# mhnazeri/PMoE

Measured on AMD Instinct MI355X. Metric: samples/sec fwd+bwd, 256x256 RGB 4-expert PMoE, higher is better.
Workload: dtype bf16; 1 GPU; 4-expert MoE (PMoE experts), 256x256x3 x4 frames, batch 64/GPU, fwd+moe_loss+bwd, dropout 0.3; global_batch=64, parallelism=dp1

## Files before the change

### include/pmoe_hip.h

```cpp
#ifndef PMOE_HIP_H
#define PMOE_HIP_H
#include <stdint.h>
#ifdef __cplusplus
extern "C" {
#endif

#define PMOE_DT_BF16 0
#define PMOE_DT_F32 1

#define PMOE_ERR_ARG (-1)
#define PMOE_ERR_UNSUPPORTED (-2)

#define PMOE_ACT_NONE 0
#define PMOE_ACT_RELU 1
#define PMOE_ACT_ELU 2
#define PMOE_ACT_TANH 3
#define PMOE_ACT_SIGMOID 4

#define PMOE_RES_NONE 0
#define PMOE_RES_ADD 1
#define PMOE_RES_DRELU 2
#define PMOE_RES_DELU 3
#define PMOE_RES_DTANH 4
#define PMOE_RES_DSIGMOID 5
#define PMOE_RES_DBN 6
#define PMOE_RES_INBN 7

#define PMOE_ABI_VERSION 401
int pmoe_version(void);
const char* pmoe_error_string(int code);
int pmoe_abi_sizeof(int which);

typedef struct pmoe_conv_desc {
    const void* in;
    const void* w;
    void* out;
    const void* res;
    const float* bias;
    float* stats;
    int32_t n, h, w_, cin;
    int32_t ho, wo, cout, coutp;
    int32_t in_ld, in_coff, out_ld, out_coff, res_ld, res_coff;
    int32_t ipe;
    int32_t in_shared;
    int32_t ks, stride, pad, dilate;
    int32_t act, res_mode;
    float drop_p;
    uint64_t seed;
    int32_t dtype;
    int32_t w_fp8;
    float in_scale;
    const float* out_scale;
    int32_t in_fp8;
    const float* bn_coef;
    int32_t bn_ipe;
    int32_t shuffle_c;
} pmoe_conv_desc;

int pmoe_conv2d_igemm(const pmoe_conv_desc* d, void* stream);
// ... 282 lines not shown
```

### pmoe_amd/csrc/elementwise.hip

```cpp
#include "common.h"

template <typename T, int MODE>
__global__ void __launch_bounds__(256) colstats_kernel(const T* __restrict__ x, const T* __restrict__ dy,
                                                      const T* __restrict__ y, const float* __restrict__ mean,
                                                      const float* __restrict__ invstd, const float* __restrict__ scale,
                                                      const float* __restrict__ shift, long long rpe, int C, int ld,
                                                      int coff, int relu, float* __restrict__ part, int nparts,
                                                      float* __restrict__ shiftc, T* __restrict__ gmask) {
    constexpr int VE = 16 / (int)sizeof(T);
    const int CV = C / VE, RL = 256 / CV;
    const int tid = threadIdx.x, cv = tid % CV, rl = tid / CV;
    const int e = blockIdx.y, pi = blockIdx.x;
    const long long rpp = (rpe + nparts - 1) / nparts;
    long long r0 = (long long)pi * rpp, r1 = r0 + rpp;
    if (r1 > rpe) r1 = rpe;
    float s1[VE], s2[VE], mu[VE], is[VE], sc[VE], sh[VE];
    const bool remask = MODE && relu && !y;
#pragma unroll
    for (int i = 0; i < VE; ++i) {
        s1[i] = s2[i] = 0.f;
        mu[i] = MODE ? mean[e * C + cv * VE + i] : 0.f;
        is[i] = MODE ? invstd[e * C + cv * VE + i] : 0.f;
        sc[i] = remask ? scale[e * C + cv * VE + i] : 0.f;
        sh[i] = remask ? shift[e * C + cv * VE + i] : 0.f;
    }
    const size_t ebase = (size_t)e * rpe;
    float c0v[VE];
#pragma unroll
    for (int i = 0; i < VE; ++i) c0v[i] = 0.f;
    if (MODE == 0 && shiftc) {
        unpack16<T>(ldg16(x + ebase * ld + coff + cv * VE), c0v);
        if (pi == 0 && rl == 0) {
#pragma unroll
            for (int i = 0; i < VE; ++i) shiftc[e * C + cv * VE + i] = c0v[i];
        }
    }
    for (long long r = r0 + rl; r < r1; r += RL) {
        const size_t off = (ebase + r) * ld + coff + cv * VE;
        float xv[VE];
        unpack16<T>(ldg16(x + off), xv);
        if (MODE == 0) {
#pragma unroll
            for (int i = 0; i < VE; ++i) { const float d = xv[i] - c0v[i]; s1[i] += d; s2[i] += d * d; }
        } else {
            float gv[VE], yv[VE];
            unpack16<T>(ldg16(dy + off), gv);
            if (remask) {
#pragma unroll
                for (int i = 0; i < VE; ++i) gv[i] = ((xv[i] - mu[i]) * sc[i] + sh[i]) > 0.f ? gv[i] : 0.f;
            } else if (relu) {
                unpack16<T>(ldg16(y + off), yv);
#pragma unroll
                for (int i = 0; i < VE; ++i) gv[i] = yv[i] > 0.f ? gv[i] : 0.f;
            }
            if (gmask) stg16(gmask + off, pack16<T>(gv));
#pragma unroll
            for (int i = 0; i < VE; ++i) { s1[i] += gv[i]; s2[i] += gv[i] * (xv[i] - mu[i]) * is[i]; }
        }
    }
    __shared__ float red[2][256 * 8 / 1];
#pragma unroll
    for (int i = 0; i < VE; ++i) {
        red[0][rl * C + cv * VE + i] = s1[i];
        red[1][rl * C + cv * VE + i] = s2[i];
    }
    __syncthreads();
    for (int c = tid; c < 2 * C; c += 256) {
        const int which = c / C, cc = c % C;
        float s = 0.f;
        for (int k = 0; k < RL; ++k) s += red[which][k * C + cc];
        part[(((size_t)e * nparts + pi) * 2 + which) * C + cc] = s;
    }
}

template <typename T>
static int colstats_launch(const void* x, const void* dy, const void* y, const float* mean, const float* invstd,
                           const float* scale, const float* shift, long long rpe, int E, int C, int ld, int coff, int relu, float* part, int nparts, int mode,
                           float* shiftc, hipStream_t st, void* gmask = nullptr) {
    if (!one_vec_per_thread<T>(C) || nparts < 1 || rpe < 1 || E < 1) return PMOE_ERR_ARG;
    if (ld <= 0) { ld = C; coff = 0; }
    if (coff < 0 || !window_ok<T>(C, ld, coff)) return PMOE_ERR_ARG;
    dim3 grid(nparts, E), block(256);
    if (mode == 0)
        return launch<colstats_kernel<T, 0>, 0>(grid, block, 0, st, (const T*)x, nullptr, nullptr, nullptr, nullptr, nullptr,
                                                nullptr, rpe, C, ld, coff, 0, part, nparts, shiftc, nullptr);
    return launch<colstats_kernel<T, 1>, 0>(grid, block, 0, st, (const T*)x, (const T*)dy, (const T*)y, mean, invstd, scale,
                                            shift, rpe, C, ld, coff, relu, part, nparts, nullptr, (T*)gmask);
}

__global__ void __launch_bounds__(256) reduce_partials_kernel(const float* __restrict__ in, float* __restrict__ out,
// ... 99 lines not shown
                                                      unsigned char* __restrict__ y8, float in_scale) {
    constexpr int VE = 16 / (int)sizeof(T);
    const int CV = C / VE;
    const int e = blockIdx.y;
    const long long nvec = rpe * CV;
    const size_t ebase = (size_t)e * rpe * C;
    const long long i0 = (long long)blockIdx.x * 256 + threadIdx.x;
    const int cv = (int)(i0 % CV);
    float sc[VE], sh[VE], mu[VE];
#pragma unroll
    for (int k = 0; k < VE; ++k) {
        sc[k] = scale[e * C + cv * VE + k]; sh[k] = shift[e * C + cv * VE + k]; mu[k] = mean[e * C + cv * VE + k];
    }
    for (long long i = i0; i < nvec; i += (long long)gridDim.x * 256) {
        float xv[VE];
        const size_t off = ebase + (size_t)i * VE;
        unpack16<T>(ldg16(x + off), xv);
#pragma unroll
        for (int k = 0; k < VE; ++k) xv[k] = (xv[k] - mu[k]) * sc[k] + sh[k];
        if (res) {
            float rv[VE];
            unpack16<T>(ldg16(res + off), rv);
#pragma unroll
            for (int k = 0; k < VE; ++k) xv[k] += rv[k];
        }
        if (relu) {
#pragma unroll
            for (int k = 0; k < VE; ++k) xv[k] = fmaxf(xv[k], 0.f);
        }
        const size_t yoff = y_ld == C ? off : ((size_t)e * rpe + (size_t)(i >> log_cv)) * y_ld + y_coff + (size_t)cv * VE;
        const v4i pk = pack16<T>(xv);
        stg16(y + yoff, pk);
        if constexpr (sizeof(T) == 2) {
            if (y8) {
                float q[VE];
                unpack16<T>(pk, q);
                int w0 = 0, w1 = 0;
#pragma unroll
                for (int k = 0; k < VE; ++k) q[k] = fminf(fmaxf(q[k] * in_scale, -PMOE_FP8_MAX), PMOE_FP8_MAX);
                w0 = __builtin_amdgcn_cvt_pk_fp8_f32(q[0], q[1], w0, false);
                w0 = __builtin_amdgcn_cvt_pk_fp8_f32(q[2], q[3], w0, true);
                w1 = __builtin_amdgcn_cvt_pk_fp8_f32(q[4], q[5], w1, false);
                w1 = __builtin_amdgcn_cvt_pk_fp8_f32(q[6], q[7], w1, true);
                *reinterpret_cast<int2*>(y8 + ebase + (size_t)i * VE) = int2{w0, w1};
            }
        }
    }
}

template <typename T>
__global__ void __launch_bounds__(256) bn_bwd_apply_kernel(const T* __restrict__ dy, const T* __restrict__ y,
                                                          const T* __restrict__ x, const float* __restrict__ mean,
                                                          const float* __restrict__ invstd,
                                                          const float* __restrict__ scale, const float* __restrict__ shift,
                                                          const float* __restrict__ c1,
                                                          const float* __restrict__ c2, T* __restrict__ dx,
                                                          T* __restrict__ gm, long long rpe, int C, int relu) {
    constexpr int VE = 16 / (int)sizeof(T);
    const int CV = C / VE;
    const int e = blockIdx.y;
    const long long nvec = rpe * CV;
    const size_t ebase = (size_t)e * rpe * C;
    const long long i0 = (long long)blockIdx.x * 256 + threadIdx.x;
    const int cv = (int)(threadIdx.x & (CV - 1));
    float A[VE], Bx[VE], K[VE], sc[VE], sh[VE], mu[VE];
#pragma unroll
    for (int k = 0; k < VE; ++k) {
        const int c = e * C + cv * VE + k;
        sc[k] = scale[c];
        sh[k] = shift ? shift[c] : 0.f;
        mu[k] = mean[c];
        A[k] = sc[k];
        Bx[k] = -sc[k] * invstd[c] * c2[c];
        K[k] = -sc[k] * c1[c];
    }
    const bool remask = relu && !y;
    for (long long i = i0; i < nvec; i += (long long)gridDim.x * 256) {
        const size_t off = ebase + (size_t)i * VE;
        float gv[VE], xv[VE], o[VE];
        unpack16<T>(ldg16(dy + off), gv);
        unpack16<T>(ldg16(x + off), xv);
        if (remask) {
#pragma unroll
            for (int k = 0; k < VE; ++k) gv[k] = ((xv[k] - mu[k]) * sc[k] + sh[k]) > 0.f ? gv[k] : 0.f;
        } else if (relu) {
            float yv[VE];
            unpack16<T>(ldg16(y + off), yv);
#pragma unroll
            for (int k = 0; k < VE; ++k) gv[k] = yv[k] > 0.f ? gv[k] : 0.f;
        }
#pragma unroll
        for (int k = 0; k < VE; ++k) o[k] = gv[k] * A[k] + ((xv[k] - mu[k]) * Bx[k] + K[k]);
        stg16(dx + off, pack16<T>(o));
        if (gm) stg16(gm + off, pack16<T>(gv));
    }
}

template <typename T>
__global__ void __launch_bounds__(256) bn_apply_pool2_kernel(const T* __restrict__ x, T* __restrict__ y, T* __restrict__ pooled,
                                                            const float* __restrict__ scale, const float* __restrict__ shift,
                                                            const float* __restrict__ mean, int ipe, int H, int W, int C, int relu,
                                                            int y_ld, int y_coff) {
    constexpr int VE = 16 / (int)sizeof(T);
    const int CV = C / VE;
    const int e = blockIdx.y, Ho = H / 2, Wo = W / 2;
    const long long nq = (long long)ipe * Ho * Wo * CV;
    const long long i0 = (long long)blockIdx.x * 256 + threadIdx.x;
    const int cv = (int)(i0 % CV);
    float sc[VE], sh[VE], mu[VE];
#pragma unroll
    for (int k = 0; k < VE; ++k) {
        sc[k] = scale[e * C + cv * VE + k]; sh[k] = shift[e * C + cv * VE + k]; mu[k] = mean[e * C + cv * VE + k];
    }
    const size_t rpe = (size_t)ipe * H * W;
    for (long long i = i0; i < nq; i += (long long)gridDim.x * 256) {
        long long t = i / CV;
        const int ox = (int)(t % Wo); t /= Wo;
// ... 389 lines not shown

template <typename T>
__global__ void __launch_bounds__(256) act_bwd_kernel(const T* __restrict__ dy, const T* __restrict__ y, T* __restrict__ dx,
                                                     long long nvec, int act, float drop_p) {
    constexpr int VE = 16 / (int)sizeof(T);
    const float keep_scale = drop_p > 0.f ? 1.f / (1.f - drop_p) : 1.f;
    const int mode = act == PMOE_ACT_ELU ? PMOE_RES_DELU : act == PMOE_ACT_TANH ? PMOE_RES_DTANH : PMOE_RES_DSIGMOID;
    for (long long i = (long long)blockIdx.x * 256 + threadIdx.x; i < nvec; i += (long long)gridDim.x * 256) {
        float g[VE], yv[VE];
        unpack16<T>(ldg16(dy + i * VE), g);
        unpack16<T>(ldg16(y + i * VE), yv);
#pragma unroll
        for (int k = 0; k < VE; ++k) {
            if (act == PMOE_ACT_NONE) g[k] = (drop_p > 0.f && yv[k] == 0.f) ? 0.f : g[k] * keep_scale;
            else if (act == PMOE_ACT_RELU) g[k] = yv[k] > 0.f ? g[k] * keep_scale : 0.f;
            else g[k] = (drop_p > 0.f && yv[k] == 0.f) ? 0.f : g[k] * act_deriv_from_output(mode, yv[k] * (1.f / keep_scale)) * keep_scale;
        }
        stg16(dx + i * VE, pack16<T>(g));
    }
}

extern "C" {

int pmoe_colstats(const void* x, int64_t rows_per_expert, int32_t E, int32_t C, int32_t ld, int32_t coff, float* part,
                  int32_t nparts, float* shiftc, int32_t dtype, void* stream) {
    DISPATCH_DT(dtype, return colstats_launch<T>(x, nullptr, nullptr, nullptr, nullptr, nullptr, nullptr, rows_per_expert, E, C, ld, coff,
                                                 0, part, nparts, 0, shiftc, (hipStream_t)stream));
}

int pmoe_bn_bwd_reduce(const void* dy, const void* y, const void* x, const float* mean, const float* invstd,
                       const float* scale, const float* shift, int64_t rows_per_expert, int32_t E, int32_t C, int32_t relu, float* part, int32_t nparts,
                       void* gmask_out, int32_t dtype, void* stream) {
    if (relu && !y && (!scale || !shift)) return PMOE_ERR_ARG;
    DISPATCH_DT(dtype, return colstats_launch<T>(x, dy, y, mean, invstd, scale, shift, rows_per_expert, E, C, C, 0, relu, part,
                                                 nparts, 1, nullptr, (hipStream_t)stream, gmask_out));
}

int pmoe_reduce_partials(const float* part_in, float* part_out, int32_t E, int32_t nin, int32_t nout, int32_t width,
                         void* stream) {
    if (nin < 1 || nout < 1 || width < 1) return PMOE_ERR_ARG;
    return launch<reduce_partials_kernel, 0>(dim3(nout, E), dim3(256), 0, (hipStream_t)stream, part_in, part_out, nin, nout, width);
}

int pmoe_bn_finalize(const float* part, int32_t nparts, int64_t count, const void* const* gamma_ptrs,
                     const void* const* beta_ptrs, void* const* rmean_ptrs, void* const* rvar_ptrs, float momentum,
                     float eps, int32_t training, float* scale, float* shift, float* mean, float* invstd, int32_t E,
                     int32_t C, const float* shiftc, void* stream) {
    if (!training && (!rmean_ptrs || !rvar_ptrs)) return PMOE_ERR_ARG;
    return launch<bn_finalize_kernel, 0>(dim3((C + FIN_CH - 1) / FIN_CH, E), dim3(FIN_CH * FIN_LANES), 0, (hipStream_t)stream,
                                         part, nparts, (long long)count, (const float* const*)gamma_ptrs,
                                         (const float* const*)beta_ptrs, (float* const*)rmean_ptrs, (float* const*)rvar_ptrs,
                                         momentum, eps, training, scale, shift, mean, invstd, C, shiftc);
}

int pmoe_bn_bwd_finalize(const float* part, int32_t nparts, int64_t count, float* dgamma, float* dbeta, float* c1,
                         float* c2, int32_t E, int32_t C, void* stream) {
    return launch<bn_bwd_finalize_kernel, 0>(dim3((C + FIN_CH - 1) / FIN_CH, E), dim3(FIN_CH * FIN_LANES), 0, (hipStream_t)stream,
                                             part, nparts, (long long)count, dgamma, dbeta, c1, c2, C);
}

int pmoe_bn_apply(const void* x, const void* res, void* y, const float* scale, const float* shift, const float* mean,
                  int64_t rows_per_expert, int32_t E, int32_t C, int32_t relu, int32_t y_ld, int32_t y_coff, int32_t dtype,
                  void* y_fp8, float in_scale, void* stream) {
    DISPATCH_DT(dtype, {
        if (!one_vec_per_thread<T>(C)) return PMOE_ERR_ARG;
        if (y_ld <= 0) { y_ld = C; y_coff = 0; }
        if (y_fp8 && (dtype != PMOE_DT_BF16 || y_ld != C)) return PMOE_ERR_ARG;
        if (!window_ok<T>(C, y_ld, y_coff)) return PMOE_ERR_ARG;
        const int CV = C / VecOf<T>::N;
        return launch<bn_apply_kernel<T>, 0>(dim3(grid_for(rows_per_expert * CV, 2048), E), dim3(256), 0, (hipStream_t)stream,
                                             (const T*)x, (const T*)res, (T*)y, scale, shift, mean, (long long)rows_per_expert, C,
                                             relu, y_ld, y_coff, ilog2_exact(CV), (unsigned char*)y_fp8, in_scale);
    });
}

int pmoe_bn_apply_pool2(const void* x, void* y, void* pooled, const float* scale, const float* shift, const float* mean,
                        int32_t ipe, int32_t H, int32_t W, int32_t E, int32_t C, int32_t relu, int32_t y_ld, int32_t y_coff,
                        int32_t dtype, void* stream) {
    if (!x || !y || !pooled || ipe < 1 || E < 1 || H < 2 || W < 2 || (H & 1) || (W & 1)) return PMOE_ERR_ARG;
    DISPATCH_DT(dtype, {
        if (!one_vec_per_thread<T>(C)) return PMOE_ERR_ARG;
        if (y_ld <= 0) { y_ld = C; y_coff = 0; }
        if (!window_ok<T>(C, y_ld, y_coff)) return PMOE_ERR_ARG;
        const long long nq = (long long)ipe * (H / 2) * (W / 2) * (C / VecOf<T>::N);
        return launch<bn_apply_pool2_kernel<T>, 0>(dim3(grid_for(nq, 2048), E), dim3(256), 0, (hipStream_t)stream, (const T*)x,
                                                   (T*)y, (T*)pooled, scale, shift, mean, ipe, H, W, C, relu, y_ld, y_coff);
    });
}

int pmoe_bn_bwd_apply(const void* dy, const void* y, const void* x, const float* mean, const float* invstd,
                      const float* scale, const float* shift, const float* c1, const float* c2, void* dx, void* gmask_out,
                      int64_t rows_per_expert, int32_t E, int32_t C, int32_t relu, int32_t dtype, void* stream) {
    DISPATCH_DT(dtype, {
        if (!one_vec_per_thread<T>(C)) return PMOE_ERR_ARG;
        const long long nvec = rows_per_expert * (C / VecOf<T>::N);
        int cap = 1024 / (E > 0 ? E : 1);
        cap = cap < 64 ? 64 : cap;
        return launch<bn_bwd_apply_kernel<T>, 0>(dim3(grid_for(nvec, cap), E), dim3(256), 0, (hipStream_t)stream, (const T*)dy,
                                                 (const T*)y, (const T*)x, mean, invstd, scale, shift, c1, c2, (T*)dx,
                                                 (T*)gmask_out, (long long)rows_per_expert, C, relu);
    });
}

int pmoe_act_fwd(const void* x, void* y, int64_t n, int32_t act, float drop_p, uint64_t seed, int32_t dtype, void* stream) {
    if (!x || !y || n <= 0 || act < PMOE_ACT_NONE || act > PMOE_ACT_SIGMOID || drop_p < 0.f || drop_p >= 1.f) return PMOE_ERR_ARG;
    DISPATCH_DT(dtype, {
        constexpr int VE = VecOf<T>::N;
        if (n % VE) return PMOE_ERR_ARG;
        return launch<act_fwd_kernel<T>, 0>(dim3(grid_for(n / VE, 4096)), dim3(256), 0, (hipStream_t)stream, (const T*)x, (T*)y,
                                            (long long)(n / VE), act, drop_p, (unsigned long long)seed);
    });
}

int pmoe_act_bwd(const void* dy, const void* y, void* dx, int64_t n, int32_t act, float drop_p, int32_t dtype, void* stream) {
    if (!dy || !y || !dx || n <= 0 || act < PMOE_ACT_NONE || act > PMOE_ACT_SIGMOID || drop_p < 0.f || drop_p >= 1.f) return PMOE_ERR_ARG;
    DISPATCH_DT(dtype, {
        constexpr int VE = VecOf<T>::N;
        if (n % VE) return PMOE_ERR_ARG;
        return launch<act_bwd_kernel<T>, 0>(dim3(grid_for(n / VE, 4096)), dim3(256), 0, (hipStream_t)stream, (const T*)dy,
                                            (const T*)y, (T*)dx, (long long)(n / VE), act, drop_p);
    });
}

int pmoe_maxpool3s2_fwd(const void* x, void* y, uint8_t* argmax, int32_t N, int32_t H, int32_t W, int32_t C,
                        int32_t dtype, void* stream) {
// ... 118 lines not shown
```

### pmoe_amd/engine.py

```python
import collections
import itertools
import os

import torch
import torch.distributed as dist

from . import hip, ops
from .model import blocks as B
from .parallel import BucketedAllReduce

F32 = torch.float32


def r16(c):
    return (c + 15) // 16 * 16


def r64(c):
    return (c + 63) // 64 * 64


class Var:
    __slots__ = ("t", "coff", "c", "g", "needs_grad", "act", "drop_p", "base", "gap_part", "bn_src", "bn_part", "f8", "bn_defer",
                 "bn_fused", "pending_bn")

    def __init__(self, t, c=None, coff=0, needs_grad=False, base=None):
        self.t, self.coff, self.c = t, coff, (c if c is not None else t.shape[-1])
        self.g, self.needs_grad, self.act, self.drop_p, self.base = None, needs_grad, hip.ACT_NONE, 0.0, base
        self.gap_part = None
        self.bn_src = None
        self.bn_part = None
        self.f8 = None
        self.bn_defer = False
        self.bn_fused = None
        self.pending_bn = None

    @property
    def grad(self):
        return self.base.g if self.base is not None else self.g

    def set_grad(self, g):
        if (self.base if self.base is not None else self).bn_part is not None:
            raise RuntimeError("relu(BatchNorm(z)) whose backward reductions came out of its consumer's data gradient "
                               "(PMOE_RES_DBN) takes exactly one consumer; a second gradient contribution arrived")
        if self.base is not None:
            self.base.g = g
        else:
            self.g = g

    def window(self, coff, c):
        v = Var(self.t, c, coff, self.needs_grad, base=self if self.base is None else self.base)
        return v


PackSinks = collections.namedtuple("PackSinks", "gen by_param")


class GroupedConv:
    scatter_grads = None
    route_bias = True

    def __init__(self, eng, name, weights, biases, cin, cout, ks, stride, pad):
        self.eng, self.name = eng, name
        self.weights, self.biases = weights, biases
        self.cin, self.cout, self.ks, self.stride, self.pad = cin, cout, ks, stride, pad
        self.cinp, self.coutp, self.cout_st = r16(cin), r64(cout), r16(cout)
        self.dg_rows, self.dg_red = r64(cin), r16(cout)
        self.taps = ks * ks
# ... 508 lines not shown
    def _bn_coeffs(self, layer, rpe, part=None, nparts=0, z=None, shiftc=None):
        E, C_ = self.E, layer.C
        coef = self._last_coef = torch.empty(4, E, C_, dtype=F32, device=self.dev)
        mean, invstd, scale, shift = coef[0], coef[1], coef[2], coef[3]
        if self.training:
            if part is None:
                nparts = self._nparts(rpe)
                part = torch.empty(E, nparts, 2, C_, dtype=F32, device=self.dev)
                shiftc = torch.empty(E, C_, dtype=F32, device=self.dev)
                ops.colstats(rpe, z.t, E, C_, part, nparts, shiftc=shiftc)
            part, nparts = self._fold_parts(part, nparts, 2 * C_, cap=2048)
            ops.bn_finalize(part, nparts, rpe, self._tab("gamma", layer), self._tab("beta", layer),
                            self._tab("rm", layer), self._tab("rv", layer), layer.momentum, layer.eps, True, scale,
                            shift, mean, invstd, E, C_, shiftc)
            self._bn_touched.append(layer)
        else:
            ops.bn_finalize(scale, 0, rpe, self._tab("gamma", layer), self._tab("beta", layer), self._tab("rm", layer),
                            self._tab("rv", layer), layer.momentum, layer.eps, False, scale, shift, mean, invstd, E, C_)
        return scale, shift, mean, invstd

    def _bn(self, z, layer, relu, res=None, stats=None, out=None, out_coff=0, want_gap=False, want_f8=False, pool_to=None):
        E, C_ = self.E, layer.C
        n, h, w, _ = z.t.shape
        rpe = self.B * h * w
        if stats is not None and stats.shape[2] != C_:
            raise RuntimeError("fused stats width mismatch")
        scale, shift, mean, invstd = self._bn_coeffs(layer, rpe, stats, stats.shape[0] // E if stats is not None else 0, z)
        if out is None:
            y = Var(torch.empty_like(z.t))
        elif self.taping:
            y = Var(out.t, C_, out_coff)
        else:
            y = out.window(out_coff, C_)
        ops.set_meta(name=layer.name, bytes=z.t.numel() * z.t.element_size() * (3 if res is not None else 2))
        if want_gap and res is None and out is None:
            nparts = self._gap_parts(h * w)
            part = torch.empty(n, nparts, C_, dtype=F32, device=self.dev)
            ops.bn_apply_gap(z.t, y.t, scale, shift, mean, part, nparts, self.B, relu)
            y.gap_part = (part, nparts)
        elif pool_to is not None and res is None:
            ops.bn_apply_pool2(z.t, y.t, pool_to, scale, shift, mean, self.B, E, C_, relu, y_coff=y.coff)
        else:
            if want_f8 and out is None and self.dtype == torch.bfloat16:
                y.f8 = torch.empty(y.t.shape, dtype=torch.uint8, device=self.dev)
            ops.bn_apply(z.t, res.t if res is not None else None, y.t, scale, shift, mean, rpe, E, C_, relu, y_coff=y.coff,
                         y_fp8=y.f8, in_scale=self.fp8_in_scale)
        if self.debug_acts is not None and relu:
            self.debug_acts[layer.name] = (y.t, y.coff, C_)
        if relu and res is None and out is None and self.taping and self.training and self.dtype == torch.bfloat16 and z.needs_grad:
            y.bn_src = (z, layer, self._last_coef, rpe)
        y.needs_grad = z.needs_grad or layer.trainable or (res is not None and res.needs_grad)
        if out is not None and y.needs_grad:
            out.needs_grad = True
        if self.taping and y.needs_grad:
            train = self.training
            self.tape.append(lambda: self._bn_bwd(z, layer, y, res, relu, scale, shift, mean, invstd, rpe, train))
        return y

    def _bn_bwd(self, z, layer, y, res, relu, scale, shift, mean, invstd, rpe, train):
        dy = y.grad
        if self.debug_grads is not None and dy is not None:
            self.debug_grads[layer.name] = dy.detach().clone()
        ysrc = y.t if (res is not None or not relu) else None
        if dy is None:
            return
        E, C_ = self.E, layer.C
        nb = z.t.numel() * z.t.element_size()
        if y.bn_part is not None:
            part, nparts = y.bn_part
            if part.shape[2] != C_:
                raise RuntimeError("BatchNorm reductions from the data-gradient epilogue: channel count mismatch")
            part, nparts = self._fold_parts(part.view(E, nparts, 2 * C_), nparts, 2 * C_, cap=2048)
            c1, c2 = self._bn_bwd_finalize(layer, part, nparts, rpe, train)
            if z.needs_grad:
                if z.grad is not None:
                    raise RuntimeError("BN input consumed twice")
                if z.bn_defer:
                    z.bn_fused = (dy, y.bn_src[2], c1, c2)
                    z.set_grad(dy)
                    return
                dz = torch.empty_like(z.t)
                ops.set_meta(name=layer.name, bytes=nb * 3)
                ops.bn_bwd_apply(dy, None, z.t, mean, invstd, scale, shift, c1, c2, dz, None, rpe, E, C_, False)
                z.set_grad(dz)
            return
        nparts = self._nparts(rpe)
        part = torch.empty(E, nparts, 2, C_, dtype=F32, device=self.dev)
        want_res = res is not None and res.needs_grad
        gm = torch.empty_like(z.t) if (want_res and relu and ysrc is not None) else None
        ops.set_meta(name=layer.name, bytes=nb * ((3 if ysrc is not None else 2) + (gm is not None)))
        ops.bn_bwd_reduce(dy, ysrc, z.t, mean, invstd, scale, shift, rpe, E, C_, relu, part, nparts, gmask=gm)
        part, nparts = self._fold_parts(part, nparts, 2 * C_, cap=2048)
        c1, c2 = self._bn_bwd_finalize(layer, part, nparts, rpe, train)
        dz = torch.empty_like(z.t) if z.needs_grad else None
        if gm is not None:
            if dz is not None:
                ops.set_meta(name=layer.name, bytes=nb * 3)
                ops.bn_bwd_apply(gm, None, z.t, mean, invstd, scale, shift, c1, c2, dz, None, rpe, E, C_, False)
        else:
            gm = torch.empty_like(z.t) if want_res else None
            if dz is None and gm is None:
                return
            if dz is None:
                dz = torch.empty_like(z.t)
            ops.set_meta(name=layer.name, bytes=nb * (2 + (ysrc is not None) + 1 + (gm is not None)))
            ops.bn_bwd_apply(dy, ysrc, z.t, mean, invstd, scale, shift, c1, c2, dz, gm, rpe, E, C_, relu)
        if self.debug_grads is not None:
            self.debug_grads[layer.name + ":dz"] = dz.detach().clone()
            self.debug_grads[layer.name + ":stats"] = (mean.clone(), invstd.clone(), c1.clone(), c2.clone())
        if z.needs_grad:
            if z.grad is not None:
                raise RuntimeError("BN input consumed twice")
            z.set_grad(dz)
        if want_res:
            if res.grad is not None:
                raise RuntimeError("residual gradient slot already filled")
            res.set_grad(gm)

    def _bn_bwd_finalize(self, layer, part, nparts, rpe, train, out=None):
        E, C_ = self.E, layer.C
        c1, c2 = out or (torch.empty(E, C_, dtype=F32, device=self.dev) for _ in range(2))
        dgamma, dbeta, store = self._bn_grad_views(layer)
        ops.bn_bwd_finalize(part, nparts, rpe, dgamma, dbeta, c1, c2, E, C_)
        if store is not None:
            store()
        if not train:
            c1.zero_()
            c2.zero_()
        return c1, c2

    def _bn_grad_views(self, layer):
        return (self._grad_slot("gamma", layer).view(self.E, layer.C), self._grad_slot("beta", layer).view(self.E, layer.C),
                None)

    def _stem_tail(self, z2, stats):
        E, C_ = self.E, self.bn_c2.C
        n, h, w, _ = z2.t.shape
        rpe = self.B * h * w
        sc2, sh2, mu2, is2 = self._bn_coeffs(self.bn_c2, rpe, stats, stats.shape[0] // E if stats is not None else 0, z2)
# ... 537 lines not shown
```

### pmoe_amd/hip.py

```python
import ctypes as C
import os
from pathlib import Path

import torch

_LIB_PATH = Path(os.environ.get("PMOE_HIP_LIB") or Path(__file__).resolve().parent / "libpmoe_hip.so")
_lib = None

ABI_VERSION = 401
DT_BF16, DT_F32 = 0, 1
ACT_NONE, ACT_RELU, ACT_ELU, ACT_TANH, ACT_SIGMOID = 0, 1, 2, 3, 4
RES_NONE, RES_ADD, RES_DRELU, RES_DELU, RES_DTANH, RES_DSIGMOID, RES_DBN, RES_INBN = 0, 1, 2, 3, 4, 5, 6, 7
ERR_ARG, ERR_UNSUPPORTED = -1, -2
RES_OF_ACT = {ACT_RELU: RES_DRELU, ACT_ELU: RES_DELU, ACT_TANH: RES_DTANH, ACT_SIGMOID: RES_DSIGMOID}
ACT_BY_NAME = {"relu": ACT_RELU, "elu": ACT_ELU, "tanh": ACT_TANH, "sigmoid": ACT_SIGMOID}

_TORCH_DT = {torch.bfloat16: DT_BF16, torch.float32: DT_F32}


class HipUnavailable(RuntimeError):
    pass


class ConvDesc(C.Structure):
    _fields_ = [
        ("in_", C.c_void_p), ("w", C.c_void_p), ("out", C.c_void_p), ("res", C.c_void_p),
        ("bias", C.c_void_p), ("stats", C.c_void_p),
        ("n", C.c_int32), ("h", C.c_int32), ("w_", C.c_int32), ("cin", C.c_int32),
        ("ho", C.c_int32), ("wo", C.c_int32), ("cout", C.c_int32), ("coutp", C.c_int32),
        ("in_ld", C.c_int32), ("in_coff", C.c_int32), ("out_ld", C.c_int32), ("out_coff", C.c_int32),
        ("res_ld", C.c_int32), ("res_coff", C.c_int32),
        ("ipe", C.c_int32), ("in_shared", C.c_int32),
        ("ks", C.c_int32), ("stride", C.c_int32), ("pad", C.c_int32), ("dilate", C.c_int32),
        ("act", C.c_int32), ("res_mode", C.c_int32),
        ("drop_p", C.c_float), ("seed", C.c_uint64), ("dtype", C.c_int32),
        ("w_fp8", C.c_int32), ("in_scale", C.c_float), ("out_scale", C.c_void_p),
        ("in_fp8", C.c_int32), ("bn_coef", C.c_void_p), ("bn_ipe", C.c_int32), ("shuffle_c", C.c_int32),
    ]


class WgradDesc(C.Structure):
    _fields_ = [
        ("x", C.c_void_p), ("dy", C.c_void_p), ("dw_ws", C.c_void_p),
        ("n", C.c_int32), ("h", C.c_int32), ("w_", C.c_int32), ("cin", C.c_int32), ("cinp", C.c_int32),
        ("ho", C.c_int32), ("wo", C.c_int32), ("cout", C.c_int32), ("coutp", C.c_int32),
        ("x_ld", C.c_int32), ("x_coff", C.c_int32), ("dy_ld", C.c_int32), ("dy_coff", C.c_int32),
# ... 210 lines not shown
```

### pmoe_amd/ops.py

```python
import ctypes as C

import torch

from . import hip
from .hip import ConvDesc, WgradDesc, check, dt, load, ptr, stream_ptr


def _round_up(v, m):
    return (v + m - 1) // m * m


def conv_out_size(h, ks, stride, pad):
    return (h + 2 * pad - ks) // stride + 1


def _nhwc(t, name):
    if t.dim() != 4:
        raise ValueError(f"{name}: expected NHWC [N,H,W,C], got shape {tuple(t.shape)}")
    return t.shape


def _conv_desc(n, h, w_, ho, wo, cin, cout, coutp, ipe, ks, stride, pad, dtype, *, dilate=False, in_shared=False, in_ld=0,
               in_coff=0, out_ld=0, out_coff=0, res_mode=hip.RES_NONE, res_ld=0, res_coff=0, act=hip.ACT_NONE, drop_p=0.0, seed=0,
               w_fp8=False, in_fp8=False, in_scale=1.0, bn_ipe=0, shuffle2_c=0):
# ... 271 lines not shown
                                stream_ptr()), "pmoe_pack_bias")


def act_fwd(x, y, act, drop_p=0.0, seed=0):
    check(load().pmoe_act_fwd(ptr(x, "x"), ptr(y, "y", x.dtype), x.numel(), act, float(drop_p), int(seed), dt(x), stream_ptr()),
          "pmoe_act_fwd")


def act_bwd(dy, y, dx, act, drop_p=0.0):
    check(load().pmoe_act_bwd(ptr(dy, "dy"), ptr(y, "y", dy.dtype), ptr(dx, "dx", dy.dtype), dy.numel(), act, float(drop_p),
                              dt(dy), stream_ptr()), "pmoe_act_bwd")


def colstats(x2d_rows_per_expert, x, E, C_, part, nparts, ld=None, coff=0, shiftc=None):
    check(load().pmoe_colstats(ptr(x, "x"), x2d_rows_per_expert, E, C_, ld if ld is not None else x.shape[-1], coff,
                               ptr(part, "part", torch.float32), nparts, ptr(shiftc, "shiftc", torch.float32), dt(x),
                               stream_ptr()), "pmoe_colstats")


def reduce_partials(part_in, part_out, E, nin, nout, width):
    check(load().pmoe_reduce_partials(ptr(part_in, "part_in", torch.float32), ptr(part_out, "part_out", torch.float32),
                                      E, nin, nout, width, stream_ptr()), "pmoe_reduce_partials")


def bn_finalize(part, nparts, count, gamma_tab, beta_tab, rmean_tab, rvar_tab, momentum, eps, training, scale, shift,
                mean, invstd, E, C_, shiftc=None):
    f32 = torch.float32
    check(load().pmoe_bn_finalize(ptr(part, "part", f32), nparts, count, ptr(gamma_tab), ptr(beta_tab), ptr(rmean_tab),
                                  ptr(rvar_tab), momentum, eps, int(training), ptr(scale, "scale", f32),
                                  ptr(shift, "shift", f32), ptr(mean, "mean", f32), ptr(invstd, "invstd", f32), E, C_,
                                  ptr(shiftc, "shiftc", f32), stream_ptr()), "pmoe_bn_finalize")


def bn_apply(x, res, y, scale, shift, mean, rpe, E, C_, relu, y_coff=0, y_fp8=None, in_scale=1.0):
    if y_fp8 is not None and (y_fp8.dtype != torch.uint8 or y_fp8.shape != y.shape):
        raise ValueError("bn_apply: y_fp8 must be a uint8 tensor of y's shape")
    check(load().pmoe_bn_apply(ptr(x, "x"), ptr(res, "res", x.dtype), ptr(y, "y", x.dtype), ptr(scale), ptr(shift),
                               ptr(mean, "mean", torch.float32), rpe,
                               E, C_, int(relu), y.shape[-1], y_coff, dt(x), ptr(y_fp8, "y_fp8", torch.uint8),
                               float(in_scale), stream_ptr()), "pmoe_bn_apply")


def bn_apply_pool2(x, y, pooled, scale, shift, mean, ipe, E, C_, relu, y_coff=0):
    n, h, w_, c = _nhwc(x, "x")
    if c != C_ or tuple(pooled.shape) != (n, h // 2, w_ // 2, C_) or tuple(y.shape[:3]) != (n, h, w_) or n != E * ipe:
        raise ValueError("bn_apply_pool2: x [E*ipe,H,W,C], y [E*ipe,H,W,ld], pooled [E*ipe,H/2,W/2,C]")
    check(load().pmoe_bn_apply_pool2(ptr(x, "x"), ptr(y, "y", x.dtype), ptr(pooled, "pooled", x.dtype), ptr(scale), ptr(shift),
                                     ptr(mean, "mean", torch.float32), ipe, h, w_, E, C_, int(relu), y.shape[-1], y_coff, dt(x),
                                     stream_ptr()), "pmoe_bn_apply_pool2")


def bn_bwd_reduce(dy, y, x, mean, invstd, scale, shift, rpe, E, C_, relu, part, nparts, gmask=None):
    check(load().pmoe_bn_bwd_reduce(ptr(dy, "dy"), ptr(y, "y", dy.dtype), ptr(x, "x", dy.dtype), ptr(mean), ptr(invstd),
                                    ptr(scale), ptr(shift), rpe, E, C_, int(relu), ptr(part, "part", torch.float32), nparts,
                                    ptr(gmask, "gmask", dy.dtype), dt(dy), stream_ptr()), "pmoe_bn_bwd_reduce")


def bn_bwd_finalize(part, nparts, count, dgamma, dbeta, c1, c2, E, C_):
    check(load().pmoe_bn_bwd_finalize(ptr(part), nparts, count, ptr(dgamma), ptr(dbeta), ptr(c1), ptr(c2), E, C_,
                                      stream_ptr()), "pmoe_bn_bwd_finalize")


def bn_bwd_apply(dy, y, x, mean, invstd, scale, shift, c1, c2, dx, gmask, rpe, E, C_, relu):
    check(load().pmoe_bn_bwd_apply(ptr(dy, "dy"), ptr(y, "y", dy.dtype), ptr(x, "x", dy.dtype), ptr(mean), ptr(invstd),
                                   ptr(scale), ptr(shift), ptr(c1), ptr(c2), ptr(dx, "dx", dy.dtype), ptr(gmask, "gmask", dy.dtype),
                                   rpe, E, C_, int(relu), dt(dy), stream_ptr()), "pmoe_bn_bwd_apply")


def stem_tail_stats(z2, sc2, sh2, mu2, part, nparts, E, ipe, shiftc=None, part_x=None):
    n, h, w_, c = _nhwc(z2, "z2")
    check(load().pmoe_stem_tail_stats(ptr(z2, "z2"), ptr(sc2), ptr(sh2), ptr(mu2), ptr(part, "part", torch.float32), nparts,
                                      ptr(shiftc, "shiftc", torch.float32), ptr(part_x, "part_x", torch.float32), E, ipe,
                                      h, w_, c, dt(z2), stream_ptr()), "pmoe_stem_tail_stats")


def _consts12(consts):
    return (C.c_void_p * 12)(*[t.data_ptr() if t is not None else None for t in consts])


def stem_tail_pooled(y, dpool, argmax, consts, part4, nparts, E):
    n, ho, wo, c = _nhwc(y, "y")
    check(load().pmoe_stem_tail_pooled(ptr(y, "y"), ptr(dpool, "dpool", y.dtype), ptr(argmax, "argmax", torch.uint8),
                                       _consts12(consts), ptr(part4, "part4", torch.float32), nparts, E,
                                       (n // E) * ho * wo, c, dt(y), stream_ptr()), "pmoe_stem_tail_pooled")


def stem_tail_combine(part4, np4, part_x, npx, consts, count, out1, out2, E, c):
    f32 = torch.float32
    check(load().pmoe_stem_tail_combine(ptr(part4, "part4", f32), np4, ptr(part_x, "part_x", f32), npx, _consts12(consts),
                                        count, ptr(out1, "out1", f32), ptr(out2, "out2", f32), E, c, stream_ptr()),
          "pmoe_stem_tail_combine")


def stem_tail_pool(z2, y, argmax, sc2, sh2, sc1, sh1, mu2, mu1, ipe):
    n, h, w_, c = _nhwc(z2, "z2")
    check(load().pmoe_stem_tail_pool(ptr(z2, "z2"), ptr(y, "y", z2.dtype), ptr(argmax, "argmax", torch.uint8), ptr(sc2),
                                     ptr(sh2), ptr(sc1), ptr(sh1), ptr(mu2), ptr(mu1), n, ipe, h, w_, c, dt(z2), stream_ptr()),
          "pmoe_stem_tail_pool")

# ... 397 lines not shown
```

Baseline: 1911 samples/s.

## Store ReLU masks as packed bits for residual BN backward

For residual BN+ReLU layers in bf16 training, the forward apply kernel now writes a 1-bit-per-channel ReLU mask, and the backward reduce and apply kernels read that mask instead of reloading the full bf16 output. This cuts backward memory traffic for the y tensor to one sixteenth, at the cost of an extra small write in forward. The colstats backward loop is also unrolled over four rows to batch loads and hide latency.

```diff
diff --git a/include/pmoe_hip.h b/include/pmoe_hip.h
--- a/include/pmoe_hip.h
+++ b/include/pmoe_hip.h
@@ -25,6 +25,8 @@
 #define PMOE_RES_DSIGMOID 5
 #define PMOE_RES_DBN 6
 #define PMOE_RES_INBN 7
+
+#define PMOE_RELU_BITS 2
 
 #define PMOE_ABI_VERSION 401
 int pmoe_version(void);
diff --git a/pmoe_amd/csrc/elementwise.hip b/pmoe_amd/csrc/elementwise.hip
--- a/pmoe_amd/csrc/elementwise.hip
+++ b/pmoe_amd/csrc/elementwise.hip
@@ -1,4 +1,6 @@
 #include "common.h"
+
+constexpr int COLSTATS_ROWS = 4;
 
 template <typename T, int MODE>
 __global__ void __launch_bounds__(256) colstats_kernel(const T* __restrict__ x, const T* __restrict__ dy,
@@ -35,27 +37,55 @@
             for (int i = 0; i < VE; ++i) shiftc[e * C + cv * VE + i] = c0v[i];
         }
     }
-    for (long long r = r0 + rl; r < r1; r += RL) {
-        const size_t off = (ebase + r) * ld + coff + cv * VE;
-        float xv[VE];
-        unpack16<T>(ldg16(x + off), xv);
-        if (MODE == 0) {
+    if constexpr (MODE == 0) {
+        for (long long r = r0 + rl; r < r1; r += RL) {
+            float xv[VE];
+            unpack16<T>(ldg16(x + (ebase + r) * ld + coff + cv * VE), xv);
 #pragma unroll
             for (int i = 0; i < VE; ++i) { const float d = xv[i] - c0v[i]; s1[i] += d; s2[i] += d * d; }
-        } else {
-            float gv[VE], yv[VE];
-            unpack16<T>(ldg16(dy + off), gv);
+        }
+    } else {
+        const bool bits = relu == PMOE_RELU_BITS, from_y = relu && !remask && !bits;
+        const unsigned char* __restrict__ yb = reinterpret_cast<const unsigned char*>(y);
+        auto add_row = [&](const v4i& xr, const v4i& gr, const v4i& yr, unsigned mb, size_t off) {
+            float xv[VE], gv[VE];
+            unpack16<T>(xr, xv);
+            unpack16<T>(gr, gv);
             if (remask) {
 #pragma unroll
                 for (int i = 0; i < VE; ++i) gv[i] = ((xv[i] - mu[i]) * sc[i] + sh[i]) > 0.f ? gv[i] : 0.f;
+            } else if (bits) {
+#pragma unroll
+                for (int i = 0; i < VE; ++i) gv[i] = ((mb >> i) & 1u) ? gv[i] : 0.f;
             } else if (relu) {
-                unpack16<T>(ldg16(y + off), yv);
+                float yv[VE];
+                unpack16<T>(yr, yv);
 #pragma unroll
                 for (int i = 0; i < VE; ++i) gv[i] = yv[i] > 0.f ? gv[i] : 0.f;
             }
             if (gmask) stg16(gmask + off, pack16<T>(gv));
 #pragma unroll
             for (int i = 0; i < VE; ++i) { s1[i] += gv[i]; s2[i] += gv[i] * (xv[i] - mu[i]) * is[i]; }
+        };
+        long long r = r0 + rl;
+        for (; r + (long long)(COLSTATS_ROWS - 1) * RL < r1; r += (long long)COLSTATS_ROWS * RL) {
+            v4i xr[COLSTATS_ROWS], gr[COLSTATS_ROWS], yr[COLSTATS_ROWS];
+            unsigned mb[COLSTATS_ROWS];
+#pragma unroll
+            for (int u = 0; u < COLSTATS_ROWS; ++u) {
+                const size_t row = ebase + r + (long long)u * RL, off = row * ld + coff + cv * VE;
+                xr[u] = ldg16(x + off);
+                gr[u] = ldg16(dy + off);
+                yr[u] = from_y ? ldg16(y + off) : v4i{0, 0, 0, 0};
+                mb[u] = bits ? yb[row * CV + cv] : 0u;
+            }
+#pragma unroll
+            for (int u = 0; u < COLSTATS_ROWS; ++u)
+                add_row(xr[u], gr[u], yr[u], mb[u], (ebase + r + (long long)u * RL) * ld + coff + cv * VE);
+        }
+        for (; r < r1; r += RL) {
+            const size_t row = ebase + r, off = row * ld + coff + cv * VE;
+            add_row(ldg16(x + off), ldg16(dy + off), from_y ? ldg16(y + off) : v4i{0, 0, 0, 0}, bits ? yb[row * CV + cv] : 0u, off);
         }
     }
     __shared__ float red[2][256 * 8 / 1];
@@ -221,7 +251,14 @@
         const v4i pk = pack16<T>(xv);
         stg16(y + yoff, pk);
         if constexpr (sizeof(T) == 2) {
-            if (y8) {
+            if (y8 && relu == PMOE_RELU_BITS) {
+                float q[VE];
+                unpack16<T>(pk, q);
+                unsigned m = 0;
+#pragma unroll
+                for (int k = 0; k < VE; ++k) m |= (q[k] > 0.f ? 1u : 0u) << k;
+                y8[(size_t)e * nvec + (size_t)i] = (unsigned char)m;
+            } else if (y8) {
                 float q[VE];
                 unpack16<T>(pk, q);
                 int w0 = 0, w1 = 0;
@@ -263,7 +300,8 @@
         Bx[k] = -sc[k] * invstd[c] * c2[c];
         K[k] = -sc[k] * c1[c];
     }
-    const bool remask = relu && !y;
+    const bool remask = relu && !y, bits = relu == PMOE_RELU_BITS;
+    const unsigned char* __restrict__ yb = reinterpret_cast<const unsigned char*>(y);
     for (long long i = i0; i < nvec; i += (long long)gridDim.x * 256) {
         const size_t off = ebase + (size_t)i * VE;
         float gv[VE], xv[VE], o[VE];
@@ -272,6 +310,10 @@
         if (remask) {
 #pragma unroll
             for (int k = 0; k < VE; ++k) gv[k] = ((xv[k] - mu[k]) * sc[k] + sh[k]) > 0.f ? gv[k] : 0.f;
+        } else if (bits) {
+            const unsigned m = yb[(size_t)e * nvec + (size_t)i];
+#pragma unroll
+            for (int k = 0; k < VE; ++k) gv[k] = ((m >> k) & 1u) ? gv[k] : 0.f;
         } else if (relu) {
             float yv[VE];
             unpack16<T>(ldg16(y + off), yv);
@@ -727,6 +769,7 @@
                        const float* scale, const float* shift, int64_t rows_per_expert, int32_t E, int32_t C, int32_t relu, float* part, int32_t nparts,
                        void* gmask_out, int32_t dtype, void* stream) {
     if (relu && !y && (!scale || !shift)) return PMOE_ERR_ARG;
+    if (relu == PMOE_RELU_BITS && (!y || dtype != PMOE_DT_BF16)) return PMOE_ERR_ARG;
     DISPATCH_DT(dtype, return colstats_launch<T>(x, dy, y, mean, invstd, scale, shift, rows_per_expert, E, C, C, 0, relu, part,
                                                  nparts, 1, nullptr, (hipStream_t)stream, gmask_out));
 }
@@ -761,6 +804,7 @@
         if (!one_vec_per_thread<T>(C)) return PMOE_ERR_ARG;
         if (y_ld <= 0) { y_ld = C; y_coff = 0; }
         if (y_fp8 && (dtype != PMOE_DT_BF16 || y_ld != C)) return PMOE_ERR_ARG;
+        if (relu == PMOE_RELU_BITS && !y_fp8) return PMOE_ERR_ARG;
         if (!window_ok<T>(C, y_ld, y_coff)) return PMOE_ERR_ARG;
         const int CV = C / VecOf<T>::N;
         return launch<bn_apply_kernel<T>, 0>(dim3(grid_for(rows_per_expert * CV, 2048), E), dim3(256), 0, (hipStream_t)stream,
@@ -786,6 +830,7 @@
 int pmoe_bn_bwd_apply(const void* dy, const void* y, const void* x, const float* mean, const float* invstd,
                       const float* scale, const float* shift, const float* c1, const float* c2, void* dx, void* gmask_out,
                       int64_t rows_per_expert, int32_t E, int32_t C, int32_t relu, int32_t dtype, void* stream) {
+    if (relu == PMOE_RELU_BITS && (!y || dtype != PMOE_DT_BF16)) return PMOE_ERR_ARG;
     DISPATCH_DT(dtype, {
         if (!one_vec_per_thread<T>(C)) return PMOE_ERR_ARG;
         const long long nvec = rows_per_expert * (C / VecOf<T>::N);
diff --git a/pmoe_amd/engine.py b/pmoe_amd/engine.py
--- a/pmoe_amd/engine.py
+++ b/pmoe_amd/engine.py
@@ -22,7 +22,7 @@
 
 class Var:
     __slots__ = ("t", "coff", "c", "g", "needs_grad", "act", "drop_p", "base", "gap_part", "bn_src", "bn_part", "f8", "bn_defer",
-                 "bn_fused", "pending_bn")
+                 "bn_fused", "pending_bn", "relu_bits")
 
     def __init__(self, t, c=None, coff=0, needs_grad=False, base=None):
         self.t, self.coff, self.c = t, coff, (c if c is not None else t.shape[-1])
@@ -34,6 +34,7 @@
         self.bn_defer = False
         self.bn_fused = None
         self.pending_bn = None
+        self.relu_bits = None
 
     @property
     def grad(self):
@@ -608,6 +609,7 @@
             y = Var(out.t, C_, out_coff)
         else:
             y = out.window(out_coff, C_)
+        needs_grad = z.needs_grad or layer.trainable or (res is not None and res.needs_grad)
         ops.set_meta(name=layer.name, bytes=z.t.numel() * z.t.element_size() * (3 if res is not None else 2))
         if want_gap and res is None and out is None:
             nparts = self._gap_parts(h * w)
@@ -619,13 +621,16 @@
         else:
             if want_f8 and out is None and self.dtype == torch.bfloat16:
                 y.f8 = torch.empty(y.t.shape, dtype=torch.uint8, device=self.dev)
+            if (res is not None and relu and self.taping and self.training and self.dtype == torch.bfloat16 and out is None
+                    and y.f8 is None and needs_grad):
+                y.relu_bits = torch.empty(y.t.shape[:-1] + (C_ // 8,), dtype=torch.uint8, device=self.dev)
             ops.bn_apply(z.t, res.t if res is not None else None, y.t, scale, shift, mean, rpe, E, C_, relu, y_coff=y.coff,
-                         y_fp8=y.f8, in_scale=self.fp8_in_scale)
+                         y_fp8=y.f8, in_scale=self.fp8_in_scale, relu_bits=y.relu_bits)
         if self.debug_acts is not None and relu:
             self.debug_acts[layer.name] = (y.t, y.coff, C_)
         if relu and res is None and out is None and self.taping and self.training and self.dtype == torch.bfloat16 and z.needs_grad:
             y.bn_src = (z, layer, self._last_coef, rpe)
-        y.needs_grad = z.needs_grad or layer.trainable or (res is not None and res.needs_grad)
+        y.needs_grad = needs_grad
         if out is not None and y.needs_grad:
             out.needs_grad = True
         if self.taping and y.needs_grad:
@@ -638,6 +643,8 @@
         if self.debug_grads is not None and dy is not None:
             self.debug_grads[layer.name] = dy.detach().clone()
         ysrc = y.t if (res is not None or not relu) else None
+        ybits = y.relu_bits if (ysrc is not None and relu) else None
+        yarg = ysrc if ybits is None else None
         if dy is None:
             return
         E, C_ = self.E, layer.C
@@ -664,8 +671,9 @@
         part = torch.empty(E, nparts, 2, C_, dtype=F32, device=self.dev)
         want_res = res is not None and res.needs_grad
         gm = torch.empty_like(z.t) if (want_res and relu and ysrc is not None) else None
-        ops.set_meta(name=layer.name, bytes=nb * ((3 if ysrc is not None else 2) + (gm is not None)))
-        ops.bn_bwd_reduce(dy, ysrc, z.t, mean, invstd, scale, shift, rpe, E, C_, relu, part, nparts, gmask=gm)
+        ybytes = 0 if ysrc is None else nb if ybits is None else ybits.numel()
+        ops.set_meta(name=layer.name, bytes=nb * (2 + (gm is not None)) + ybytes)
+        ops.bn_bwd_reduce(dy, yarg, z.t, mean, invstd, scale, shift, rpe, E, C_, relu, part, nparts, gmask=gm, y_bits=ybits)
         part, nparts = self._fold_parts(part, nparts, 2 * C_, cap=2048)
         c1, c2 = self._bn_bwd_finalize(layer, part, nparts, rpe, train)
         dz = torch.empty_like(z.t) if z.needs_grad else None
@@ -679,8 +687,8 @@
                 return
             if dz is None:
                 dz = torch.empty_like(z.t)
-            ops.set_meta(name=layer.name, bytes=nb * (2 + (ysrc is not None) + 1 + (gm is not None)))
-            ops.bn_bwd_apply(dy, ysrc, z.t, mean, invstd, scale, shift, c1, c2, dz, gm, rpe, E, C_, relu)
+            ops.set_meta(name=layer.name, bytes=nb * (3 + (gm is not None)) + ybytes)
+            ops.bn_bwd_apply(dy, yarg, z.t, mean, invstd, scale, shift, c1, c2, dz, gm, rpe, E, C_, relu, y_bits=ybits)
         if self.debug_grads is not None:
             self.debug_grads[layer.name + ":dz"] = dz.detach().clone()
             self.debug_grads[layer.name + ":stats"] = (mean.clone(), invstd.clone(), c1.clone(), c2.clone())
diff --git a/pmoe_amd/hip.py b/pmoe_amd/hip.py
--- a/pmoe_amd/hip.py
+++ b/pmoe_amd/hip.py
@@ -12,6 +12,7 @@
 ACT_NONE, ACT_RELU, ACT_ELU, ACT_TANH, ACT_SIGMOID = 0, 1, 2, 3, 4
 RES_NONE, RES_ADD, RES_DRELU, RES_DELU, RES_DTANH, RES_DSIGMOID, RES_DBN, RES_INBN = 0, 1, 2, 3, 4, 5, 6, 7
 ERR_ARG, ERR_UNSUPPORTED = -1, -2
+RELU_BITS = 2
 RES_OF_ACT = {ACT_RELU: RES_DRELU, ACT_ELU: RES_DELU, ACT_TANH: RES_DTANH, ACT_SIGMOID: RES_DSIGMOID}
 ACT_BY_NAME = {"relu": ACT_RELU, "elu": ACT_ELU, "tanh": ACT_TANH, "sigmoid": ACT_SIGMOID}
 
diff --git a/pmoe_amd/ops.py b/pmoe_amd/ops.py
--- a/pmoe_amd/ops.py
+++ b/pmoe_amd/ops.py
@@ -327,12 +327,27 @@
                                   ptr(shiftc, "shiftc", f32), stream_ptr()), "pmoe_bn_finalize")
 
 
-def bn_apply(x, res, y, scale, shift, mean, rpe, E, C_, relu, y_coff=0, y_fp8=None, in_scale=1.0):
+def _relu_arg(relu, bits, other, what):
+    if bits is None:
+        return int(relu)
+    if other is not None or not relu:
+        raise ValueError(f"{what}: the ReLU bits go with relu=True and take the place of the other tensor of their slot")
+    if bits.dtype != torch.uint8:
+        raise ValueError(f"{what}: the ReLU bits are a uint8 tensor")
+    return hip.RELU_BITS
+
+
+def bn_apply(x, res, y, scale, shift, mean, rpe, E, C_, relu, y_coff=0, y_fp8=None, in_scale=1.0, relu_bits=None):
     if y_fp8 is not None and (y_fp8.dtype != torch.uint8 or y_fp8.shape != y.shape):
         raise ValueError("bn_apply: y_fp8 must be a uint8 tensor of y's shape")
+    relu_arg = _relu_arg(relu, relu_bits, y_fp8, "bn_apply")
+    if relu_bits is not None:
+        if x.dtype != torch.bfloat16 or tuple(relu_bits.shape) != tuple(y.shape[:-1]) + (C_ // 8,):
+            raise ValueError("bn_apply: relu_bits needs bfloat16 data and a uint8 tensor of shape y.shape[:-1] + (C // 8,)")
+        y_fp8 = relu_bits
     check(load().pmoe_bn_apply(ptr(x, "x"), ptr(res, "res", x.dtype), ptr(y, "y", x.dtype), ptr(scale), ptr(shift),
                                ptr(mean, "mean", torch.float32), rpe,
-                               E, C_, int(relu), y.shape[-1], y_coff, dt(x), ptr(y_fp8, "y_fp8", torch.uint8),
+                               E, C_, relu_arg, y.shape[-1], y_coff, dt(x), ptr(y_fp8, "y_fp8", torch.uint8),
                                float(in_scale), stream_ptr()), "pmoe_bn_apply")
 
 
@@ -345,9 +360,19 @@
                                      stream_ptr()), "pmoe_bn_apply_pool2")
 
 
-def bn_bwd_reduce(dy, y, x, mean, invstd, scale, shift, rpe, E, C_, relu, part, nparts, gmask=None):
-    check(load().pmoe_bn_bwd_reduce(ptr(dy, "dy"), ptr(y, "y", dy.dtype), ptr(x, "x", dy.dtype), ptr(mean), ptr(invstd),
-                                    ptr(scale), ptr(shift), rpe, E, C_, int(relu), ptr(part, "part", torch.float32), nparts,
+def _y_slot(y, y_bits, dy, relu, what):
+    relu_arg = _relu_arg(relu, y_bits, y, what)
+    if y_bits is None:
+        return ptr(y, "y", dy.dtype), relu_arg
+    if dy.dtype != torch.bfloat16 or tuple(y_bits.shape) != tuple(dy.shape[:-1]) + (dy.shape[-1] // 8,):
+        raise ValueError(f"{what}: y_bits needs bfloat16 data and a uint8 tensor of shape dy.shape[:-1] + (C // 8,)")
+    return ptr(y_bits, "y_bits", torch.uint8), relu_arg
+
+
+def bn_bwd_reduce(dy, y, x, mean, invstd, scale, shift, rpe, E, C_, relu, part, nparts, gmask=None, y_bits=None):
+    yp, relu_arg = _y_slot(y, y_bits, dy, relu, "bn_bwd_reduce")
+    check(load().pmoe_bn_bwd_reduce(ptr(dy, "dy"), yp, ptr(x, "x", dy.dtype), ptr(mean), ptr(invstd),
+                                    ptr(scale), ptr(shift), rpe, E, C_, relu_arg, ptr(part, "part", torch.float32), nparts,
                                     ptr(gmask, "gmask", dy.dtype), dt(dy), stream_ptr()), "pmoe_bn_bwd_reduce")
 
 
@@ -356,10 +381,11 @@
                                       stream_ptr()), "pmoe_bn_bwd_finalize")
 
 
-def bn_bwd_apply(dy, y, x, mean, invstd, scale, shift, c1, c2, dx, gmask, rpe, E, C_, relu):
-    check(load().pmoe_bn_bwd_apply(ptr(dy, "dy"), ptr(y, "y", dy.dtype), ptr(x, "x", dy.dtype), ptr(mean), ptr(invstd),
+def bn_bwd_apply(dy, y, x, mean, invstd, scale, shift, c1, c2, dx, gmask, rpe, E, C_, relu, y_bits=None):
+    yp, relu_arg = _y_slot(y, y_bits, dy, relu, "bn_bwd_apply")
+    check(load().pmoe_bn_bwd_apply(ptr(dy, "dy"), yp, ptr(x, "x", dy.dtype), ptr(mean), ptr(invstd),
                                    ptr(scale), ptr(shift), ptr(c1), ptr(c2), ptr(dx, "dx", dy.dtype), ptr(gmask, "gmask", dy.dtype),
-                                   rpe, E, C_, int(relu), dt(dy), stream_ptr()), "pmoe_bn_bwd_apply")
+                                   rpe, E, C_, relu_arg, dt(dy), stream_ptr()), "pmoe_bn_bwd_apply")
 
 
 def stem_tail_stats(z2, sc2, sh2, mu2, part, nparts, E, ipe, shiftc=None, part_x=None):
```

Measured after the change: 1930 samples/s (median of 6 runs). Within noise of the previous version (+1.0%).
